# zhangrengang/SubPhaser

Measured on AMD Instinct MI355X. Metric: genome Gbases/s k-mer+enrichment, wheat k=15 1Mb windows, higher is better.
Workload: dtype u32

## Files before the change

### subphaser_amd/csrc/sp_map.h

```cpp
#pragma once
#include "sp_device.h"

#ifndef MAP_BLOOM_MAX_BITS
#define MAP_BLOOM_MAX_BITS 25
#endif
#ifndef MAP_BLOOM_MIN_BITS
#define MAP_BLOOM_MIN_BITS 12
#endif
#ifndef MAP_FILL_MAX
#define MAP_FILL_MAX 0.40
#endif
#define MAP_BLOOM_CORE 0x100
#define MAP_BLOOM_NBITS(nb) ((nb) & 0xFF)
#define MAP_RUNS 0x200
#ifndef MAP_RUNS_R
#define MAP_RUNS_R 2
#endif
#ifndef MAP_RUNS_P
#define MAP_RUNS_P 3
#endif
struct map_bloom_probe {
    uint32_t word, bits;
};
__host__ __device__ __forceinline__ uint32_t map_core_hash(uint64_t t) {
    uint32_t x = (uint32_t)t ^ (uint32_t)(t >> 32);
    x *= 0x9E3779B1u;
    x ^= x >> 15;
    return x * 0x85EBCA6Bu;
}
__host__ __device__ __forceinline__ uint32_t map_core_word(uint32_t hmin , int nbits) {
    const uint32_t n = ~hmin;
    const uint32_t sq = (uint32_t)(((unsigned long long)n * (unsigned long long)n) >> 32);
    return (~sq) >> (32 - (MAP_BLOOM_NBITS(nbits) - 5));
}
__host__ __device__ __forceinline__ uint32_t map_bloom_bits3(uint64_t x64, uint32_t &h) {
    const uint32_t x = (uint32_t)x64 ^ (uint32_t)(x64 >> 32);
    h = x * 0x9E3779B1u;
    const uint32_t h2 = x * 0x85EBCA6Bu;
    return (1u << ((h >> 7) & 31u)) | (1u << ((h >> 2) & 31u)) | (1u << (h2 >> 27));
}
__host__ __device__ __forceinline__ map_bloom_probe map_bloom(uint64_t x64, int k, int nbits) {
    map_bloom_probe p;
    uint32_t h;
    p.bits = map_bloom_bits3(x64, h);
    if (!(nbits & MAP_BLOOM_CORE) || k < 5) {
        p.word = h >> (32 - (MAP_BLOOM_NBITS(nbits) - 5));
        return p;
    }
    const int cb = 2 * (k - 3);
    const uint64_t smask = (1ULL << cb) - 1ULL;
    const uint64_t a = x64 >> 4, b = x64 & smask;
    const uint64_t ar = sp_revcomp(a, k - 3), br = sp_revcomp(b, k - 3);
    const uint32_t ha = map_core_hash(a < ar ? a : ar), hb = map_core_hash(b < br ? b : br);
    p.word = map_core_word(ha < hb ? ha : hb, nbits);
    return p;
}
__device__ __forceinline__ bool map_bloom_test(const uint32_t *__restrict__ bloom, int nbits, int k, uint64_t x) {
    const map_bloom_probe p = map_bloom(x, k, nbits);
    return (bloom[p.word] & p.bits) == p.bits;
}

template <typename KeyT, typename KP, typename F>
__device__ __forceinline__ void map_pair_scan(const uint32_t *__restrict__ pk, const uint32_t *__restrict__ nm,
                                              int64_t s0, const KP &kp, const uint32_t *__restrict__ bloom,
                                              int nbits, F &&hit) {
    bool pairhit = false;
    const KeyT m1mask = (KeyT)(kp.kmask >> 2);
    sp_scan_unit_all<SP_UNIT, KeyT>(pk, nm, s0, kp, [&](int64_t start, KeyT fwd, KeyT rc, bool valid_k, bool valid_k1) {
        if (!(start & 1)) {
            pairhit = false;
            if (valid_k1) {
                const KeyT mf = fwd & m1mask, mr = rc >> 2;
                pairhit = map_bloom_test(bloom, nbits, kp.k, (uint64_t)(mf < mr ? mf : mr));
            }
        }
        if (pairhit && valid_k) hit(start, fwd, rc);
    });
}

#define MAP_PAIR_MAX_SG 7

struct map_pair_loc {
    uint32_t idx;
    int field;
};
__host__ __device__ __forceinline__ map_pair_loc map_pair_loc_prefix(uint64_t o, int k) {
    map_pair_loc r;
    const uint32_t b = (uint32_t)(o & 3ULL);
    if (k == 1) { r.idx = 0; r.field = 4 + (int)b; return r; }
    const uint64_t p = o >> 2, pc = sp_revcomp(p, k - 1);
    if (p <= pc) { r.idx = (uint32_t)p; r.field = 4 + (int)b; }
    else { r.idx = (uint32_t)pc; r.field = 3 - (int)b; }
    return r;
}
__host__ __device__ __forceinline__ map_pair_loc map_pair_loc_suffix(uint64_t o, int k) {
    map_pair_loc r;
    const uint32_t b = (uint32_t)(o >> (2 * (k - 1))) & 3u;
    if (k == 1) { r.idx = 0; r.field = (int)b; return r; }
    const uint64_t m1mask = (1ULL << (2 * (k - 1))) - 1ULL;
    const uint64_t x = o & m1mask, xc = sp_revcomp(x, k - 1);
    if (x <= xc) { r.idx = (uint32_t)x; r.field = (int)b; }
    else { r.idx = (uint32_t)xc; r.field = 7 - (int)b; }
    return r;
}

#define MAP_CT_FIELD 3
#define MAP_CT_ANY 0x6DB6DBu
#define MAP_CT_PAYLOAD 0xFFFFFFu
#define MAP_CT_OVF (1u << 24)
#define MAP_CT_MAX_TAG_BITS 2
struct map_ptab {
    uint32_t *direct;
    uint4 *buckets;
    unsigned long long *ovf;
    uint32_t ovf_mask;
    int sb, tb;
};
__host__ __device__ __forceinline__ uint32_t map_ct_mix(uint32_t x, int kb) {
    const uint32_t m = kb >= 32 ? 0xFFFFFFFFu : ((1u << kb) - 1u);
    uint32_t h = (x * 0x9E3779B1u) & m;
    h ^= h >> ((kb + 1) / 2);
    h = (h * 0x85EBCA6Bu) & m;
    h ^= h >> ((kb + 1) / 2);
    return h;
}
__host__ __device__ __forceinline__ uint32_t map_ct_ovf_home(uint32_t x) { return (x * 0xC2B2AE35u) >> 7; }
struct map_ct_key {
    uint32_t bucket, tag, kid;
};
__host__ __device__ __forceinline__ map_ct_key map_ct_key_of(const map_ptab &T, uint32_t t, uint32_t side, uint32_t e) {
    const uint32_t h = map_ct_mix(t, T.sb);
    map_ct_key r;
    r.bucket = h >> T.tb;
    r.tag = ((h & ((1u << T.tb) - 1u)) << 5) | (side << 4) | e;
    r.kid = (t << 5) | (side << 4) | e;
    return r;
}
struct map_ct_hit {
    uint32_t fields, loc;
};
__device__ __forceinline__ map_ct_hit map_ct_find(const map_ptab &T, const uint4 &B, const map_ct_key &q) {
    map_ct_hit r;
// ... 129 lines not shown
```

### subphaser_amd/csrc/sp_map.hip

```cpp
#include "sp_device.h"
#include "sp_internal.h"
#include "sp_map.h"

__global__ void __launch_bounds__(256)
k4_pair_filter(const unsigned long long *__restrict__ keys, int64_t n, int k, uint32_t *__restrict__ bloom, int nbits) {
    int64_t i = (int64_t)blockIdx.x * blockDim.x + threadIdx.x;
    if (i >= n) return;
    const uint64_t key = keys[i];
    uint64_t pre = 0, suf = 0;
    if (k > 1) {
        const uint64_t m1mask = (k - 1 >= 32) ? ~0ULL : ((1ULL << (2 * (k - 1))) - 1ULL);
        pre = key >> 2;
        suf = key & m1mask;
        const uint64_t rpre = sp_revcomp(pre, k - 1), rsuf = sp_revcomp(suf, k - 1);
        pre = pre < rpre ? pre : rpre;
        suf = suf < rsuf ? suf : rsuf;
    }
    const map_bloom_probe p = map_bloom(pre, k, nbits);
    atomicOr(&bloom[p.word], p.bits);
    const map_bloom_probe q = map_bloom(suf, k, nbits);
    atomicOr(&bloom[q.word], q.bits);
}

__global__ void __launch_bounds__(256)
k4_filter_fill(const uint32_t *__restrict__ bloom, int64_t n_words, unsigned long long *__restrict__ out) {
    __shared__ unsigned long long red[16];
    unsigned long long c = 0;
    for (int64_t i = (int64_t)blockIdx.x * blockDim.x + threadIdx.x; i < n_words; i += (int64_t)gridDim.x * blockDim.x)
        c += __popc(bloom[i]);
    unsigned long long t = sp_block_sum_u64(c, red);
    if (threadIdx.x == 0 && t) atomicAdd(out, t);
}

__global__ void __launch_bounds__(256)
k4_labels(const unsigned long long *__restrict__ keys, const uint8_t *__restrict__ sg, int64_t n,
          sp_kparams kp, uint8_t *__restrict__ label) {
    int64_t i = (int64_t)blockIdx.x * blockDim.x + threadIdx.x;
    if (i >= n) return;
    label[sp_slot_of_key(keys[i], kp)] = (uint8_t)(1u + sg[i]);
}

__global__ void __launch_bounds__(256)
k4_pair_table(const unsigned long long *__restrict__ keys, const uint8_t *__restrict__ sg, int64_t n, int k,
              uint32_t *__restrict__ ptab) {
    int64_t i = (int64_t)blockIdx.x * blockDim.x + threadIdx.x;
    if (i >= n) return;
    const uint64_t key = keys[i];
    const uint32_t l = 1u + sg[i];
    const map_pair_loc a = map_pair_loc_prefix(key, k), b = map_pair_loc_suffix(key, k);
    atomicOr(&ptab[a.idx], l << (4 * a.field));
    atomicOr(&ptab[b.idx], l << (4 * b.field));
    const uint64_t r = sp_revcomp(key, k);
    const map_pair_loc c = map_pair_loc_prefix(r, k), d = map_pair_loc_suffix(r, k);
    atomicOr(&ptab[c.idx], l << (4 * c.field));
    atomicOr(&ptab[d.idx], l << (4 * d.field));
}

__global__ void __launch_bounds__(256)
k4_pair_clear(const unsigned long long *__restrict__ keys, int64_t n, int k, uint32_t *__restrict__ ptab) {
    int64_t i = (int64_t)blockIdx.x * blockDim.x + threadIdx.x;
    if (i >= n) return;
    const uint64_t key = keys[i], r = sp_revcomp(key, k);
    ptab[map_pair_loc_prefix(key, k).idx] = 0u;
    ptab[map_pair_loc_suffix(key, k).idx] = 0u;
    ptab[map_pair_loc_prefix(r, k).idx] = 0u;
    ptab[map_pair_loc_suffix(r, k).idx] = 0u;
}

__global__ void __launch_bounds__(256)
k4_pair_seen(const unsigned long long *__restrict__ keys, int64_t n, int k, const uint32_t *__restrict__ ptab,
             unsigned long long *__restrict__ out) {
    __shared__ unsigned long long red[16];
    unsigned long long c = 0;
    for (int64_t i = (int64_t)blockIdx.x * blockDim.x + threadIdx.x; i < n; i += (int64_t)gridDim.x * blockDim.x) {
        const uint64_t key = keys[i], r = sp_revcomp(key, k);
        const map_pair_loc a = map_pair_loc_prefix(key, k), b = map_pair_loc_suffix(key, k);
        const map_pair_loc e = map_pair_loc_prefix(r, k), f = map_pair_loc_suffix(r, k);
        const uint32_t seen = ((ptab[a.idx] >> (4 * a.field)) | (ptab[b.idx] >> (4 * b.field)) |
                               (ptab[e.idx] >> (4 * e.field)) | (ptab[f.idx] >> (4 * f.field))) & 8u;
        c += seen ? 1 : 0;
    }
    unsigned long long t = sp_block_sum_u64(c, red);
    if (threadIdx.x == 0 && t) atomicAdd(out, t);
}

__device__ __forceinline__ void map_ct_insert(const map_ptab &T, const map_ct_key &q, uint32_t bits, unsigned long long *fail) {
    uint32_t *e = reinterpret_cast<uint32_t *>(T.buckets + q.bucket);
    const uint32_t fresh = (q.tag << 25) | bits;
    for (int j = 0; j < 4; j++) {
        const int i = (int)((q.tag + (uint32_t)j) & 3u);
        const uint32_t old = atomicCAS(&e[i], 0u, fresh);
        if (old == 0u) return;
        if ((old >> 25) == q.tag && (old & MAP_CT_PAYLOAD)) {
            atomicOr(&e[i], bits);
            return;
        }
    }
    atomicOr(&e[0], MAP_CT_OVF);
    const unsigned long long mine = ((unsigned long long)(q.kid + 1u) << 32) | bits;
    uint32_t i = map_ct_ovf_home(q.kid) & T.ovf_mask;
    for (uint32_t probes = 0; probes <= T.ovf_mask; probes++) {
        const unsigned long long old = atomicCAS(&T.ovf[i], 0ULL, mine);
        if (old == 0ULL) {
            atomicAdd(fail + 1, 1ULL);
// ... 26 lines not shown
    __shared__ unsigned long long red[16];
    unsigned long long c = 0;
    for (int64_t i = (int64_t)blockIdx.x * blockDim.x + threadIdx.x; i < n; i += (int64_t)gridDim.x * blockDim.x) {
        const uint64_t o2[2] = {keys[i], sp_revcomp(keys[i], k)};
        uint32_t seen = 0;
        for (int r = 0; r < 2; r++) {
            map_ct_site st[4];
            const int ns = map_ct_sites(o2[r], k, st);
            for (int j = 0; j < ns; j++) {
                const map_ct_key q = map_ct_key_of(T, st[j].t, st[j].side, st[j].e);
                const uint4 B = T.buckets[q.bucket];
                seen |= (map_ct_find(T, B, q).fields >> (MAP_CT_FIELD * st[j].field)) & 4u;
            }
        }
        c += seen ? 1 : 0;
    }
    unsigned long long t = sp_block_sum_u64(c, red);
    if (threadIdx.x == 0 && t) atomicAdd(out, t);
}

struct map_chrom_desc {
    const uint32_t *pk, *pm, *nm;
    int64_t n_units;
    int64_t nslots;
    int64_t range0;
    int *counts;
    unsigned long long *n_mapped;
};

#ifndef MAP_MIN_WAVES
#define MAP_MIN_WAVES 8
#endif
#ifndef MAP2_QI
#define MAP2_QI 1
#endif
struct map_quad_win {
    uint32_t V1, V2, xf1, xr1, xf2, xr2;
};
__device__ __forceinline__ map_quad_win map_quad_windows(uint32_t l0, uint32_t l1, uint32_t m0, uint32_t m1, int r ,
                                                         int sh, uint32_t m1mask) {
    map_quad_win q;
    const uint32_t W1 = __builtin_amdgcn_alignbit(l1, l0, 2 * r), W2 = __builtin_amdgcn_alignbit(l1, l0, 2 * r + 4);
    const unsigned long long mm = ((unsigned long long)m0 << 32) | m1;
    q.V1 = (uint32_t)((mm << (2 * r)) >> 32);
    q.V2 = (uint32_t)((mm << (2 * r + 4)) >> 32);
    q.xf1 = (q.V1 >> sh) & m1mask;
    q.xr1 = (~W1 >> 2) & m1mask;
    q.xf2 = (q.V2 >> sh) & m1mask;
    q.xr2 = (~W2 >> 2) & m1mask;
    return q;
}
template <int TABLE>
__device__ __forceinline__ void map_unit_scan64(const uint32_t *__restrict__ pk, const uint32_t *__restrict__ pm,
                                                const uint32_t *__restrict__ nm, int64_t s0, const sp_kparams32 &kp,
                                                const uint32_t *__restrict__ bloom, int nbits, const map_ptab &T,
                                                unsigned long long lab[3], const map_unit_lds &U,
                                                unsigned long long cm = ~0ULL ) {
    constexpr int FW = TABLE ? MAP_CT_FIELD : 4;
    constexpr uint32_t LBL = TABLE ? 3u : 7u, SEEN = TABLE ? 4u : 8u, FMASK = TABLE ? 7u : 15u;
    constexpr uint32_t ANY = TABLE ? MAP_CT_ANY : 0x77777777u;
    constexpr int NP = TABLE ? 2 : 3, ROUND_W = TABLE ? MAP2_ROUND_W : 2;
    unsigned long long ok_k, ok_x;
    {
        const uint64_t badA = sp_bad_starts64(nm, s0, kp.k - 1), badB = sp_bad_starts64(nm, s0 + 32, kp.k - 1);
        const uint64_t invA = (uint64_t)nm[s0 >> 5] | ((uint64_t)nm[(s0 >> 5) + 1] << 32);
        const uint64_t invB = (uint64_t)nm[(s0 >> 5) + 1] | ((uint64_t)nm[(s0 >> 5) + 2] << 32);
        const uint32_t kA = ~(uint32_t)(badA | (invA >> (kp.k - 1))), kB = ~(uint32_t)(badB | (invB >> (kp.k - 1)));
        const uint32_t xA = ~(uint32_t)(badA >> 1), xB = ~(uint32_t)(badB >> 1);
        ok_k = (unsigned long long)kA | ((unsigned long long)kB << 32);
        ok_x = (unsigned long long)xA | ((unsigned long long)xB << 32);
    }
    if (__all((ok_x & 0x5555555555555555ULL) == 0)) return;
    const unsigned long long here = __ballot(1);
    const int n_here = __popcll(here);
    const int me = (int)__builtin_amdgcn_mbcnt_hi((uint32_t)(here >> 32), __builtin_amdgcn_mbcnt_lo((uint32_t)here, 0u));
    const int tid = (int)threadIdx.x, lane = tid & 63, wave0 = tid & ~63;
    uint32_t *sw = U.words + tid;
    uint16_t *queue = U.queue + (tid >> 6) * MAP_QCAP(TABLE);
    const int64_t w0 = s0 >> 4;
    const uint4 la = *reinterpret_cast<const uint4 *>(pk + w0);
    uint32_t l0 = la.x, l1 = la.y, l2 = la.z, l3 = la.w, l4 = pk[w0 + 4];
#if SP_DERIVE_PM
    (void)pm;
    uint32_t m0 = sp_msb_of_lsb(l0), m1 = sp_msb_of_lsb(l1), m2 = sp_msb_of_lsb(l2), m3 = sp_msb_of_lsb(l3), m4 = sp_msb_of_lsb(l4);
#else
    const uint4 ma = *reinterpret_cast<const uint4 *>(pm + w0);
    uint32_t m0 = ma.x, m1 = ma.y, m2 = ma.z, m3 = ma.w, m4 = pm[w0 + 4];
#endif
    {
        const unsigned long long okc = ok_k & cm;
        sw[0 * MAP_BLOCK] = l0; sw[1 * MAP_BLOCK] = l1; sw[2 * MAP_BLOCK] = l2; sw[3 * MAP_BLOCK] = l3; sw[4 * MAP_BLOCK] = l4;
        sw[5 * MAP_BLOCK] = (uint32_t)okc; sw[6 * MAP_BLOCK] = (uint32_t)(okc >> 32);
#pragma unroll
        for (int bit = 0; bit < NP; bit++) U.planes[bit * MAP_BLOCK + tid] = 0ULL;
    }
    const int sh = 32 - 2 * kp.k, sh1 = 30 - 2 * kp.k;
    const uint32_t m1mask = kp.kmask >> 2;
    const int sb = T.sb;
    const uint32_t smask = TABLE ? ((1u << sb) - 1u) : 0u;
    const bool core = (nbits & MAP_BLOOM_CORE) && kp.k >= 5;
    const uint32_t cmask = kp.k >= 5 ? ((1u << (2 * (kp.k - 3))) - 1u) : 0u;
    const int wsh = 32 - (MAP_BLOOM_NBITS(nbits) - 5);
    uint32_t last_wi = 0xFFFFFFFFu, last_w = 0u;
    uint32_t h_carry = 0u;
    static_assert(MAP2_QI == 1, "the runs rule decides a quad from the filter's answer for the quad before it");
    const bool runs = (nbits & MAP_RUNS) != 0;
    uint32_t run = 0u;
#pragma unroll 1
    for (int wr = 0; wr < 4; wr += ROUND_W) {
        uint32_t qn = 0;
#pragma unroll 1
        for (int w = wr; w < wr + ROUND_W; w++) {
#pragma unroll 1
            for (int r0 = 0; r0 < 16; r0 += 4 * MAP2_QI) {
                uint32_t bt1[MAP2_QI], bt2[MAP2_QI], wi1[MAP2_QI], wi2[MAP2_QI], f1[MAP2_QI], f2[MAP2_QI];
                bool v1[MAP2_QI], v2[MAP2_QI], need1[MAP2_QI], need2[MAP2_QI], guess[MAP2_QI];
                uint32_t lw = last_wi;
#pragma unroll
                for (int q = 0; q < MAP2_QI; q++) {
                    const int r = r0 + 4 * q, j = 16 * w + r;
                    const map_quad_win Q = map_quad_windows(l0, l1, m0, m1, r, sh, m1mask);
                    const uint32_t c1 = Q.xf1 < Q.xr1 ? Q.xf1 : Q.xr1, c2 = Q.xf2 < Q.xr2 ? Q.xf2 : Q.xr2;
                    uint32_t h1, h2;
                    bt1[q] = map_bloom_bits3((uint64_t)c1, h1);
                    bt2[q] = map_bloom_bits3((uint64_t)c2, h2);
                    const uint32_t okx = (uint32_t)(ok_x >> j);
                    v1[q] = okx & 1u;
                    v2[q] = okx & 4u;
                    if (core) {
                        const uint32_t tb_f = Q.xf1 & cmask, tb_r = Q.xr1 >> 4, tc_f = Q.xf2 & cmask, tc_r = Q.xr2 >> 4;
                        uint32_t ha = h_carry;
                        if (j == 0) {
                            const uint32_t ta_f = Q.xf1 >> 4, ta_r = Q.xr1 & cmask;
                            ha = map_core_hash((uint64_t)(ta_f < ta_r ? ta_f : ta_r));
                        }
                        const uint32_t hb = map_core_hash((uint64_t)(tb_f < tb_r ? tb_f : tb_r));
                        const uint32_t hc = map_core_hash((uint64_t)(tc_f < tc_r ? tc_f : tc_r));
                        h_carry = hc;
                        wi1[q] = map_core_word(ha < hb ? ha : hb, nbits);
                        wi2[q] = map_core_word(hb < hc ? hb : hc, nbits);
                    } else {
                        wi1[q] = h1 >> wsh;
                        wi2[q] = h2 >> wsh;
                    }
                    guess[q] = runs && v1[q] && v2[q] && run - (uint32_t)MAP_RUNS_R < (uint32_t)MAP_RUNS_P;
                    need1[q] = !guess[q] && v1[q] && wi1[q] != lw;
                    need2[q] = !guess[q] && v2[q] && wi2[q] != (v1[q] ? wi1[q] : lw);
                    f1[q] = f2[q] = 0;
                    if (need1[q]) f1[q] = bloom[wi1[q]];
                    if (need2[q]) f2[q] = bloom[wi2[q]];
                    if (!guess[q]) {
                        if (v2[q]) lw = wi2[q];
                        else if (v1[q]) lw = wi1[q];
                    }
                }
                last_wi = lw;
#pragma unroll
                for (int q = 0; q < MAP2_QI; q++) {
                    const int j = 16 * w + r0 + 4 * q;
                    const uint32_t wd1 = v1[q] ? (need1[q] ? f1[q] : last_w) : 0u;
                    const uint32_t wd2 = v2[q] ? (need2[q] ? f2[q] : (v1[q] ? wd1 : last_w)) : 0u;
                    if (!guess[q]) {
                        if (v2[q]) last_w = wd2;
                        else if (v1[q]) last_w = wd1;
                    }
                    const bool cand1 = guess[q] || (wd1 & bt1[q]) == bt1[q], cand2 = guess[q] || (wd2 & bt2[q]) == bt2[q];
                    run = guess[q] ? run + 1u : (cand1 && cand2) ? (run < (uint32_t)MAP_RUNS_R ? run + 1u : (uint32_t)MAP_RUNS_R) : 0u;
                    const unsigned long long bal = __ballot(cand1 || cand2);
                    if (cand1 || cand2)
                        queue[qn + __builtin_amdgcn_mbcnt_hi((uint32_t)(bal >> 32), __builtin_amdgcn_mbcnt_lo((uint32_t)bal, 0u))] =
                            (uint16_t)((uint32_t)lane | ((uint32_t)(j >> 2) << 6) | (cand1 ? 0x400u : 0u) | (cand2 ? 0x800u : 0u));
                    qn += (uint32_t)__popcll(bal);
                }
            }
            l0 = l1; l1 = l2; l2 = l3; l3 = l4;
            m0 = m1; m1 = m2; m2 = m3; m3 = m4;
        }
        __builtin_amdgcn_fence(__ATOMIC_RELEASE, "wavefront");
        __builtin_amdgcn_wave_barrier();
        __builtin_amdgcn_fence(__ATOMIC_ACQUIRE, "wavefront");
        for (uint32_t e0 = (uint32_t)me; e0 < qn; e0 += (uint32_t)(MAP2_P2 * n_here)) {
            bool live[MAP2_P2], cand1[MAP2_P2], cand2[MAP2_P2], sfw[MAP2_P2];
            int owner[MAP2_P2], jj[MAP2_P2];
            map_quad_win Q[MAP2_P2];
            uint32_t okk[MAP2_P2], e1[MAP2_P2], e2[MAP2_P2];
            map_ct_key k1[MAP2_P2], k2[MAP2_P2];
            uint4 B[MAP2_P2];
#pragma unroll
            for (int p = 0; p < MAP2_P2; p++) {
                const uint32_t e = e0 + (uint32_t)(p * n_here);
                live[p] = e < qn;
                const uint32_t ent = live[p] ? (uint32_t)queue[e] : 0u;
                const int qi = (int)((ent >> 6) & 15u), w = qi >> 2;
                owner[p] = wave0 + (int)(ent & 63u);
                jj[p] = 4 * qi;
                cand1[p] = ent & 0x400u;
                cand2[p] = ent & 0x800u;
                const uint32_t *ow = U.words + owner[p];
                const uint32_t ola = ow[w * MAP_BLOCK], olb = ow[(w + 1) * MAP_BLOCK];
                Q[p] = map_quad_windows(ola, olb, sp_msb_of_lsb(ola), sp_msb_of_lsb(olb), jj[p] & 15, sh, m1mask);
                okk[p] = ow[(5 + (w >> 1)) * MAP_BLOCK] >> (jj[p] & 31);
                e1[p] = e2[p] = 0;
                sfw[p] = false;
                B[p] = make_uint4(0u, 0u, 0u, 0u);
                if (TABLE) {
                    const uint32_t s_f = cand1[p] ? (Q[p].xf1 & smask) : (Q[p].xf2 >> 4), s_r = cand1[p] ? (Q[p].xr1 >> 4) : (Q[p].xr2 & smask);
                    sfw[p] = s_f <= s_r;
                    const uint32_t t = sfw[p] ? s_f : s_r;
                    k1[p] = map_ct_key_of(T, t, sfw[p] ? 0u : 1u, sfw[p] ? (Q[p].xf1 >> sb) : (Q[p].xr1 & 15u));
                    k2[p] = map_ct_key_of(T, t, sfw[p] ? 1u : 0u, sfw[p] ? (Q[p].xf2 & 15u) : (Q[p].xr2 >> sb));
                    if (live[p]) B[p] = T.buckets[k1[p].bucket];
                } else {
                    if (cand1[p]) e1[p] = T.direct[Q[p].xf1 < Q[p].xr1 ? Q[p].xf1 : Q[p].xr1];
                    if (cand2[p]) e2[p] = T.direct[Q[p].xf2 < Q[p].xr2 ? Q[p].xf2 : Q[p].xr2];
                }
            }
#pragma unroll
            for (int p = 0; p < MAP2_P2; p++) {
                if (!live[p]) continue;
                const int j = jj[p];
                uint32_t loc1 = Q[p].xf1 < Q[p].xr1 ? Q[p].xf1 : Q[p].xr1, loc2 = Q[p].xf2 < Q[p].xr2 ? Q[p].xf2 : Q[p].xr2;
                bool fw1 = Q[p].xf1 <= Q[p].xr1, fw2 = Q[p].xf2 <= Q[p].xr2;
                if (TABLE) {
                    if (cand1[p]) {
                        const map_ct_hit h = map_ct_find(T, B[p], k1[p]);
                        e1[p] = h.fields;
                        loc1 = h.loc;
                    }
                    if (cand2[p]) {
                        const map_ct_hit h = map_ct_find(T, B[p], k2[p]);
                        e2[p] = h.fields;
                        loc2 = h.loc;
                    }
                    fw1 = fw2 = sfw[p];
                }
#pragma unroll
                for (int h = 0; h < 2; h++) {
                    const uint32_t ee = h ? e2[p] : e1[p];
                    if (!(ee & ANY)) continue;
                    const uint32_t V = h ? Q[p].V2 : Q[p].V1;
                    const bool fw = h ? fw2 : fw1;
                    const uint32_t b0 = V >> 30, b1 = (V >> sh1) & 3u;
                    const int f0 = fw ? (int)b0 : 7 - (int)b0, f1 = fw ? 4 + (int)b1 : 3 - (int)b1;
                    const uint32_t cnt2 = okk[p] >> (2 * h);
                    const uint32_t v0 = (cnt2 & 1u) ? (ee >> (FW * f0)) & FMASK : 0u;
                    const uint32_t v1 = (cnt2 & 2u) ? (ee >> (FW * f1)) & FMASK : 0u;
                    const uint32_t two = (v0 & LBL) | ((v1 & LBL) << 8);
                    if (!two) continue;
#pragma unroll
                    for (int bit = 0; bit < NP; bit++) {
                        const unsigned long long b2 = (unsigned long long)(((two >> bit) & 1u) | (((two >> (8 + bit)) & 1u) << 1));
                        if (b2) atomicOr(&U.planes[bit * MAP_BLOCK + owner[p]], b2 << (j + 2 * h));
                    }
                    uint32_t mark = 0;
                    if ((v0 & LBL) && !(v0 & SEEN)) mark |= SEEN << (FW * f0);
                    if ((v1 & LBL) && !(v1 & SEEN)) mark |= SEEN << (FW * f1);
                    if (mark) {
                        if (TABLE) map_ct_mark(T, h ? loc2 : loc1, mark);
                        else atomicOr(&T.direct[h ? loc2 : loc1], mark);
// ... 977 lines not shown
```

### subphaser_amd/csrc/sp_sparse.hip

```cpp
#include <algorithm>
#include <cstring>
#include <utility>
#include <rocprim/rocprim.hpp>

#include "sp_device.h"
#include "sp_internal.h"
#include "sp_lists.h"
#include "sp_map.h"

__global__ void __launch_bounds__(256)
sps_keygen(const uint32_t *__restrict__ pk, const uint32_t *__restrict__ nm, int64_t n_units, sp_kparams kp,
           unsigned long long *__restrict__ keys ,
           unsigned long long *__restrict__ n_valid) {
    __shared__ unsigned long long red[16];
    unsigned long long nv = 0;
    for (int64_t u = (int64_t)blockIdx.x * blockDim.x + threadIdx.x; u < n_units;
         u += (int64_t)gridDim.x * blockDim.x) {
        sp_scan_unit64<SP_UNIT>(pk, nm, u * SP_UNIT, kp, [&](int64_t start, uint64_t fwd, uint64_t rc) {
            keys[start] = fwd < rc ? fwd : rc;
            nv++;
        });
    }
    unsigned long long t = sp_block_sum_u64(nv, red);
    if (threadIdx.x == 0 && t) atomicAdd(n_valid, t);
// ... 328 lines not shown
    unsigned long long c = 0;
    for (int64_t i = (int64_t)blockIdx.x * blockDim.x + threadIdx.x; i < n; i += (int64_t)gridDim.x * blockDim.x) {
        const uint64_t o2[2] = {keys[i], sp_revcomp(keys[i], k)};
        uint32_t seen = 0;
        for (int r = 0; r < 2; r++) {
            sq_site st[4];
            const int ns = sq_sites(o2[r], k, st);
            for (int j = 0; j < ns; j++) {
                const sq_key q = sq_key_of(T, st[j].t, st[j].side, st[j].e);
                const ulonglong2 *bp = reinterpret_cast<const ulonglong2 *>(T.buckets + 4 * q.bucket);
                seen |= (sq_find(T, bp[0], bp[1], q.bucket, q.tag, st[j].t, (st[j].side << 4) | st[j].e).fields >> (SQ_FIELD * st[j].field)) & 4u;
            }
        }
        c += seen ? 1 : 0;
    }
    const unsigned long long t = sp_block_sum_u64(c, red);
    if (threadIdx.x == 0 && t) atomicAdd(out, t);
}

struct map_pair_win {
    uint64_t xf, xr;
    uint32_t b0, b1;
};
__device__ __forceinline__ map_pair_win map_pair_window(uint32_t la, uint32_t lb, uint32_t lc, uint32_t ma, uint32_t mb, uint32_t mc,
                                                        int rr, int k, int sh, uint64_t m1mask) {
    map_pair_win q;
    const uint64_t W = (uint64_t)__builtin_amdgcn_alignbit(lb, la, 2 * rr) | ((uint64_t)__builtin_amdgcn_alignbit(lc, lb, 2 * rr) << 32);
    const unsigned long long mA = ((unsigned long long)ma << 32) | mb, mB = ((unsigned long long)mb << 32) | mc;
    const uint64_t V = (((mA << (2 * rr)) >> 32) << 32) | ((mB << (2 * rr)) >> 32);
    q.b0 = (uint32_t)(V >> 62);
    q.xf = (V >> sh) & m1mask;
    q.xr = (~W >> 2) & m1mask;
    const int pb = rr + k;
    q.b1 = (((pb >> 4) == 1 ? lb : lc) >> (2 * (pb & 15))) & 3u;
    return q;
}
template <int TABLE>
__device__ __forceinline__ void map_unit_scan64_h(const uint32_t *__restrict__ pk, const uint32_t *__restrict__ pm,
                                                  const uint32_t *__restrict__ nm, int64_t s0, const sp_kparams &kp,
                                                  const uint32_t *__restrict__ bloom, int nbits,
                                                  unsigned long long *__restrict__ htab, uint64_t hmask, const sq_tab &T,
                                                  unsigned long long lab[3], const map_unit_lds &U,
                                                  unsigned long long cm = ~0ULL ) {
    constexpr int FW = TABLE ? SQ_FIELD : 4;
    constexpr uint32_t LBL = TABLE ? 3u : 7u, SEEN = TABLE ? 4u : 8u, FMASK = TABLE ? 7u : 15u;
    constexpr uint32_t ANY = TABLE ? (uint32_t)SQ_ANY : 0x77777777u;
    constexpr int NP = TABLE ? 2 : 3, ROUND_W = TABLE ? MAP2_ROUND_W : 2;
    unsigned long long ok_k, ok_x;
    {
        const uint64_t badA = sp_bad_starts64(nm, s0, kp.k - 1), badB = sp_bad_starts64(nm, s0 + 32, kp.k - 1);
        const uint64_t invA = (uint64_t)nm[s0 >> 5] | ((uint64_t)nm[(s0 >> 5) + 1] << 32);
        const uint64_t invB = (uint64_t)nm[(s0 >> 5) + 1] | ((uint64_t)nm[(s0 >> 5) + 2] << 32);
        const uint32_t kA = ~(uint32_t)(badA | (invA >> (kp.k - 1))), kB = ~(uint32_t)(badB | (invB >> (kp.k - 1)));
        const uint32_t xA = ~(uint32_t)(badA >> 1), xB = ~(uint32_t)(badB >> 1);
        ok_k = ((unsigned long long)kA | ((unsigned long long)kB << 32)) & cm;
        ok_x = (unsigned long long)xA | ((unsigned long long)xB << 32);
    }
    if (__all((ok_x & 0x5555555555555555ULL) == 0)) return;
    const unsigned long long here = __ballot(1);
    const int n_here = __popcll(here);
    const int me = (int)__builtin_amdgcn_mbcnt_hi((uint32_t)(here >> 32), __builtin_amdgcn_mbcnt_lo((uint32_t)here, 0u));
    const int tid = (int)threadIdx.x, lane = tid & 63, wave0 = tid & ~63;
    uint32_t *sw = U.words + tid;
    uint16_t *queue = U.queue + (tid >> 6) * MAP_QCAP(TABLE);
    const int64_t w0 = s0 >> 4;
    const uint4 la = *reinterpret_cast<const uint4 *>(pk + w0);
    uint32_t l0 = la.x, l1 = la.y, l2 = la.z, l3 = la.w, l4 = pk[w0 + 4], l5 = pk[w0 + 5];
#if SP_DERIVE_PM
    (void)pm;
    uint32_t m0 = sp_msb_of_lsb(l0), m1 = sp_msb_of_lsb(l1), m2 = sp_msb_of_lsb(l2), m3 = sp_msb_of_lsb(l3), m4 = sp_msb_of_lsb(l4),
             m5 = sp_msb_of_lsb(l5);
#else
    const uint4 ma = *reinterpret_cast<const uint4 *>(pm + w0);
    uint32_t m0 = ma.x, m1 = ma.y, m2 = ma.z, m3 = ma.w, m4 = pm[w0 + 4], m5 = pm[w0 + 5];
#endif
    sw[0 * MAP_BLOCK] = l0; sw[1 * MAP_BLOCK] = l1; sw[2 * MAP_BLOCK] = l2; sw[3 * MAP_BLOCK] = l3; sw[4 * MAP_BLOCK] = l4; sw[5 * MAP_BLOCK] = l5;
    sw[6 * MAP_BLOCK] = (uint32_t)ok_k; sw[7 * MAP_BLOCK] = (uint32_t)(ok_k >> 32);
#pragma unroll
    for (int bit = 0; bit < NP; bit++) U.planes[bit * MAP_BLOCK + tid] = 0ULL;
    const int sh = 64 - 2 * kp.k;
    const uint64_t m1mask = kp.kmask >> 2;
    const bool core = (nbits & MAP_BLOOM_CORE) != 0;
    const uint64_t cmask = (1ULL << (2 * (kp.k - 3))) - 1ULL;
    const int wsh = 32 - (MAP_BLOOM_NBITS(nbits) - 5);
    uint32_t last_wi = 0xFFFFFFFFu, last_w = 0u;
    uint32_t h_carry = 0u;
#pragma unroll 1
    for (int wr = 0; wr < 4; wr += ROUND_W) {
        uint32_t qn = 0;
#pragma unroll 1
        for (int w = wr; w < wr + ROUND_W; w++) {
#pragma unroll 1
            for (int r = 0; r < 16; r += 4) {
                const int j = 16 * w + r;
                const map_pair_win A = map_pair_window(l0, l1, l2, m0, m1, m2, r, kp.k, sh, m1mask);
                const map_pair_win B = map_pair_window(l0, l1, l2, m0, m1, m2, r + 2, kp.k, sh, m1mask);
                uint32_t hx1, hx2;
                const uint32_t bt1 = map_bloom_bits3(A.xf < A.xr ? A.xf : A.xr, hx1), bt2 = map_bloom_bits3(B.xf < B.xr ? B.xf : B.xr, hx2);
                uint32_t wi1, wi2;
                if (core) {
                    const uint64_t tb_f = A.xf & cmask, tb_r = A.xr >> 4, tc_f = B.xf & cmask, tc_r = B.xr >> 4;
                    uint32_t ha = h_carry;
                    if (j == 0) {
                        const uint64_t ta_f = A.xf >> 4, ta_r = A.xr & cmask;
                        ha = map_core_hash(ta_f < ta_r ? ta_f : ta_r);
                    }
                    const uint32_t hb = map_core_hash(tb_f < tb_r ? tb_f : tb_r), hc = map_core_hash(tc_f < tc_r ? tc_f : tc_r);
                    h_carry = hc;
                    wi1 = map_core_word(ha < hb ? ha : hb, nbits);
                    wi2 = map_core_word(hb < hc ? hb : hc, nbits);
                } else {
                    wi1 = hx1 >> wsh;
                    wi2 = hx2 >> wsh;
                }
                const bool v1 = (ok_x >> j) & 1ULL, v2 = (ok_x >> (j + 2)) & 1ULL;
                const bool need1 = v1 && wi1 != last_wi;
                const bool need2 = v2 && wi2 != (v1 ? wi1 : last_wi);
                uint32_t f1 = 0, f2 = 0;
                if (need1) f1 = bloom[wi1];
                if (need2) f2 = bloom[wi2];
                const uint32_t wd1 = v1 ? (need1 ? f1 : last_w) : 0u;
                const uint32_t wd2 = v2 ? (need2 ? f2 : (v1 ? wd1 : last_w)) : 0u;
                if (v2) { last_wi = wi2; last_w = wd2; }
                else if (v1) { last_wi = wi1; last_w = wd1; }
                const bool cand1 = (wd1 & bt1) == bt1, cand2 = (wd2 & bt2) == bt2;
                const unsigned long long bal = __ballot(cand1 || cand2);
                if (cand1 || cand2)
                    queue[qn + __builtin_amdgcn_mbcnt_hi((uint32_t)(bal >> 32), __builtin_amdgcn_mbcnt_lo((uint32_t)bal, 0u))] =
                        (uint16_t)((uint32_t)lane | ((uint32_t)(j >> 2) << 6) | (cand1 ? 0x400u : 0u) | (cand2 ? 0x800u : 0u));
                qn += (uint32_t)__popcll(bal);
            }
            l0 = l1; l1 = l2; l2 = l3; l3 = l4; l4 = l5;
            m0 = m1; m1 = m2; m2 = m3; m3 = m4; m4 = m5;
        }
        __builtin_amdgcn_fence(__ATOMIC_RELEASE, "wavefront");
        __builtin_amdgcn_wave_barrier();
        __builtin_amdgcn_fence(__ATOMIC_ACQUIRE, "wavefront");
        for (uint32_t e0 = (uint32_t)me; e0 < qn; e0 += (uint32_t)n_here) {
            const uint32_t ent = queue[e0];
            const int owner = wave0 + (int)(ent & 63u), qi = (int)((ent >> 6) & 15u), j = 4 * qi, w = qi >> 2, r = j & 15;
            const bool cand[2] = {(ent & 0x400u) != 0u, (ent & 0x800u) != 0u};
            const uint32_t *ow = U.words + owner;
            const uint32_t oa = ow[w * MAP_BLOCK], ob = ow[(w + 1) * MAP_BLOCK], oc = ow[(w + 2) * MAP_BLOCK];
            const uint32_t okq = ow[(6 + (w >> 1)) * MAP_BLOCK] >> (j & 31);
            const uint32_t pa = sp_msb_of_lsb(oa), pb_ = sp_msb_of_lsb(ob), pc = sp_msb_of_lsb(oc);
            const map_pair_win Pw[2] = {map_pair_window(oa, ob, oc, pa, pb_, pc, r, kp.k, sh, m1mask),
                                        map_pair_window(oa, ob, oc, pa, pb_, pc, r + 2, kp.k, sh, m1mask)};
            uint32_t e[2] = {0u, 0u};
            uint32_t loc[2] = {0u, 0u};
            uint64_t slot[2] = {0, 0};
            bool fwd_[2] = {Pw[0].xf <= Pw[0].xr, Pw[1].xf <= Pw[1].xr};
            if (TABLE) {
                const uint64_t s_f = cand[0] ? (Pw[0].xf & cmask) : (Pw[1].xf >> 4), s_r = cand[0] ? (Pw[0].xr >> 4) : (Pw[1].xr & cmask);
                const bool sfw = s_f <= s_r;
                const uint64_t t = sfw ? s_f : s_r;
                const uint64_t hm = sq_mix(t, T.sb);
                const uint64_t bucket = hm >> T.tb, tagb = (hm & ((1ULL << T.tb) - 1ULL)) << 5;
                const uint32_t se1 = (sfw ? 0u : 16u) | (uint32_t)(sfw ? (Pw[0].xf >> T.sb) : (Pw[0].xr & 15ULL));
                const uint32_t se2 = (sfw ? 16u : 0u) | (uint32_t)(sfw ? (Pw[1].xf & 15ULL) : (Pw[1].xr >> T.sb));
                const ulonglong2 *bp = reinterpret_cast<const ulonglong2 *>(T.buckets + 4 * bucket);
                const ulonglong2 B0 = bp[0], B1 = bp[1];
                if (cand[0]) {
                    const sq_hit hh = sq_find(T, B0, B1, bucket, tagb | se1, t, se1);
                    e[0] = hh.fields;
                    loc[0] = hh.loc;
                }
                if (cand[1]) {
                    const sq_hit hh = sq_find(T, B0, B1, bucket, tagb | se2, t, se2);
                    e[1] = hh.fields;
                    loc[1] = hh.loc;
                }
                fwd_[0] = fwd_[1] = sfw;
            } else {
#pragma unroll
                for (int h = 0; h < 2; h++)
                    if (cand[h]) e[h] = sps_pair_get(Pw[h].xf < Pw[h].xr ? Pw[h].xf : Pw[h].xr, htab, hmask, slot[h]);
            }
#pragma unroll
            for (int h = 0; h < 2; h++) {
                if (!(e[h] & ANY)) continue;
                const bool fw = fwd_[h];
                const int f0 = fw ? (int)Pw[h].b0 : 7 - (int)Pw[h].b0, f1 = fw ? 4 + (int)Pw[h].b1 : 3 - (int)Pw[h].b1;
                const uint32_t okk = okq >> (2 * h);
                const uint32_t v0 = (okk & 1u) ? (e[h] >> (FW * f0)) & FMASK : 0u;
                const uint32_t v1 = (okk & 2u) ? (e[h] >> (FW * f1)) & FMASK : 0u;
                const uint32_t two = (v0 & LBL) | ((v1 & LBL) << 8);
                if (!two) continue;
#pragma unroll
                for (int bit = 0; bit < NP; bit++) {
                    const unsigned long long b2 = (unsigned long long)(((two >> bit) & 1u) | (((two >> (8 + bit)) & 1u) << 1));
                    if (b2) atomicOr(&U.planes[bit * MAP_BLOCK + owner], b2 << (j + 2 * h));
                }
                uint32_t mark = 0;
                if ((v0 & LBL) && !(v0 & SEEN)) mark |= SEEN << (FW * f0);
                if ((v1 & LBL) && !(v1 & SEEN)) mark |= SEEN << (FW * f1);
                if (mark) {
                    if (TABLE) sq_mark(T, loc[h], mark);
                    else atomicOr(&htab[2 * slot[h] + 1], (unsigned long long)mark);
                }
            }
        }
        __builtin_amdgcn_fence(__ATOMIC_RELEASE, "wavefront");
        __builtin_amdgcn_wave_barrier();
        __builtin_amdgcn_fence(__ATOMIC_ACQUIRE, "wavefront");
    }
#pragma unroll
    for (int bit = 0; bit < NP; bit++) lab[bit] = U.planes[bit * MAP_BLOCK + tid];
}
// ... 649 lines not shown
```

Baseline: 156.8.

## Generalise blocked Bloom filter to configurable 32/64/128-bit blocks

Moves the Bloom filter helpers into a shared header and lets the block size (32, 64 or 128 bits) and number of hash bits per key be chosen at compile time. Wider blocks are loaded with vector loads and filled with 64-bit atomics, and the fill limit scales with the hash count. The intent is a lower false-positive rate at the same memory, so fewer candidates reach the exact lookup stage. The default stays a 32-bit block, and the derived-msb path now computes the msb plane on the fly per step instead of precomputing five registers, which cuts register pressure.

```diff
diff --git a/subphaser_amd/csrc/sp_bloom.h b/subphaser_amd/csrc/sp_bloom.h
--- /dev/null
+++ b/subphaser_amd/csrc/sp_bloom.h
@@ -0,0 +1,114 @@
+#pragma once
+#include <stdint.h>
+#if defined(__HIPCC__)
+#define SP_BLOOM_HD __host__ __device__ __forceinline__
+#else
+#define SP_BLOOM_HD static inline
+#endif
+
+#ifndef MAP_BLOOM_MAX_BITS
+#define MAP_BLOOM_MAX_BITS 25
+#endif
+#ifndef MAP_BLOOM_MIN_BITS
+#define MAP_BLOOM_MIN_BITS 12
+#endif
+#ifndef MAP_BLOOM_BLOCK
+#define MAP_BLOOM_BLOCK 32
+#endif
+#ifndef MAP_BLOOM_K
+#define MAP_BLOOM_K (MAP_BLOOM_BLOCK == 32 ? 3 : MAP_BLOOM_BLOCK == 64 ? 4 : 5)
+#endif
+#define MAP_BLOOM_LOG (MAP_BLOOM_BLOCK == 32 ? 5 : MAP_BLOOM_BLOCK == 64 ? 6 : 7)
+#define MAP_BLOOM_WORDS (MAP_BLOOM_BLOCK / 32)
+static_assert(MAP_BLOOM_BLOCK == 32 || MAP_BLOOM_BLOCK == 64 || MAP_BLOOM_BLOCK == 128, "MAP_BLOOM_BLOCK: 32, 64 or 128");
+static_assert(MAP_BLOOM_BLOCK == 32 ? MAP_BLOOM_K == 3 : (MAP_BLOOM_K == 4 || MAP_BLOOM_K == 5), "MAP_BLOOM_K: 3 at 32 bits, 4 or 5 above");
+static_assert(MAP_BLOOM_MIN_BITS > MAP_BLOOM_LOG && MAP_BLOOM_MAX_BITS - MAP_BLOOM_LOG < 32, "block index: 1 .. 31 bits");
+#ifndef MAP_FILL_MAX
+#define MAP_FILL_MAX (MAP_BLOOM_K == 3 ? 0.40 : MAP_BLOOM_K == 4 ? 0.494 : 0.573)
+#endif
+#define MAP_BLOOM_CORE 0x100
+#define MAP_BLOOM_NBITS(nb) ((nb) & 0xFF)
+
+struct map_bloom_blk {
+    uint32_t w[MAP_BLOOM_WORDS];
+};
+struct map_bloom_probe {
+    uint32_t block;
+    map_bloom_blk bits;
+};
+SP_BLOOM_HD bool map_bloom_pass(const map_bloom_blk &have, const map_bloom_blk &want) {
+    bool ok = true;
+    for (int i = 0; i < MAP_BLOOM_WORDS; i++) ok = ok && (have.w[i] & want.w[i]) == want.w[i];
+    return ok;
+}
+SP_BLOOM_HD uint64_t map_bloom_revcomp(uint64_t x, int k) {
+    x = ~x;
+    x = ((x >> 2) & 0x3333333333333333ULL) | ((x & 0x3333333333333333ULL) << 2);
+    x = ((x >> 4) & 0x0F0F0F0F0F0F0F0FULL) | ((x & 0x0F0F0F0F0F0F0F0FULL) << 4);
+    x = ((x >> 8) & 0x00FF00FF00FF00FFULL) | ((x & 0x00FF00FF00FF00FFULL) << 8);
+    x = ((x >> 16) & 0x0000FFFF0000FFFFULL) | ((x & 0x0000FFFF0000FFFFULL) << 16);
+    x = (x >> 32) | (x << 32);
+    return x >> (64 - 2 * k);
+}
+SP_BLOOM_HD uint32_t map_core_hash(uint64_t t) {
+    uint32_t x = (uint32_t)t ^ (uint32_t)(t >> 32);
+    x *= 0x9E3779B1u;
+    x ^= x >> 15;
+    return x * 0x85EBCA6Bu;
+}
+SP_BLOOM_HD uint32_t map_core_word(uint32_t hmin , int nbits) {
+    const uint32_t n = ~hmin;
+    const uint32_t sq = (uint32_t)(((unsigned long long)n * (unsigned long long)n) >> 32);
+    return (~sq) >> (32 - (MAP_BLOOM_NBITS(nbits) - MAP_BLOOM_LOG));
+}
+SP_BLOOM_HD uint32_t map_hash_word(uint32_t h, int nbits) { return h >> (32 - (MAP_BLOOM_NBITS(nbits) - MAP_BLOOM_LOG)); }
+SP_BLOOM_HD uint32_t map_bloom_sel(uint64_t x64, uint32_t &h) {
+    const uint32_t x = (uint32_t)x64 ^ (uint32_t)(x64 >> 32);
+    h = x * 0x9E3779B1u;
+    const uint32_t h2 = x * 0x85EBCA6Bu;
+#if MAP_BLOOM_BLOCK == 32
+    return (1u << ((h >> 7) & 31u)) | (1u << ((h >> 2) & 31u)) | (1u << (h2 >> 27));
+#else
+    return h2;
+#endif
+}
+SP_BLOOM_HD map_bloom_blk map_bloom_mask(uint32_t sel) {
+    map_bloom_blk b;
+#if MAP_BLOOM_BLOCK == 32
+    b.w[0] = sel;
+#elif MAP_BLOOM_BLOCK == 64
+    b.w[0] = (1u << (sel >> 28)) | (0x10000u << ((sel >> 24) & 15u));
+#if MAP_BLOOM_K == 4
+    b.w[1] = (1u << ((sel >> 20) & 15u)) | (0x10000u << ((sel >> 16) & 15u));
+#else
+    b.w[1] = (1u << ((sel >> 20) & 15u)) | (0x10000u << ((sel >> 17) & 7u)) | (0x1000000u << ((sel >> 14) & 7u));
+#endif
+#else
+    b.w[0] = 1u << (sel >> 27);
+    b.w[1] = 1u << ((sel >> 22) & 31u);
+    b.w[2] = 1u << ((sel >> 17) & 31u);
+#if MAP_BLOOM_K == 4
+    b.w[3] = 1u << ((sel >> 12) & 31u);
+#else
+    b.w[3] = (1u << ((sel >> 13) & 15u)) | (0x10000u << ((sel >> 9) & 15u));
+#endif
+#endif
+    return b;
+}
+SP_BLOOM_HD map_bloom_blk map_bloom_bits(uint64_t x64, uint32_t &h) { return map_bloom_mask(map_bloom_sel(x64, h)); }
+SP_BLOOM_HD map_bloom_probe map_bloom(uint64_t x64, int k, int nbits) {
+    map_bloom_probe p;
+    uint32_t h;
+    p.bits = map_bloom_bits(x64, h);
+    if (!(nbits & MAP_BLOOM_CORE) || k < 5) {
+        p.block = map_hash_word(h, nbits);
+        return p;
+    }
+    const int cb = 2 * (k - 3);
+    const uint64_t smask = (1ULL << cb) - 1ULL;
+    const uint64_t a = x64 >> 4, b = x64 & smask;
+    const uint64_t ar = map_bloom_revcomp(a, k - 3), br = map_bloom_revcomp(b, k - 3);
+    const uint32_t ha = map_core_hash(a < ar ? a : ar), hb = map_core_hash(b < br ? b : br);
+    p.block = map_core_word(ha < hb ? ha : hb, nbits);
+    return p;
+}
diff --git a/subphaser_amd/csrc/sp_map.h b/subphaser_amd/csrc/sp_map.h
--- a/subphaser_amd/csrc/sp_map.h
+++ b/subphaser_amd/csrc/sp_map.h
@@ -1,17 +1,7 @@
 #pragma once
 #include "sp_device.h"
-
-#ifndef MAP_BLOOM_MAX_BITS
-#define MAP_BLOOM_MAX_BITS 25
-#endif
-#ifndef MAP_BLOOM_MIN_BITS
-#define MAP_BLOOM_MIN_BITS 12
-#endif
-#ifndef MAP_FILL_MAX
-#define MAP_FILL_MAX 0.40
-#endif
-#define MAP_BLOOM_CORE 0x100
-#define MAP_BLOOM_NBITS(nb) ((nb) & 0xFF)
+#include "sp_bloom.h"
+
 #define MAP_RUNS 0x200
 #ifndef MAP_RUNS_R
 #define MAP_RUNS_R 2
@@ -19,45 +9,22 @@
 #ifndef MAP_RUNS_P
 #define MAP_RUNS_P 3
 #endif
-struct map_bloom_probe {
-    uint32_t word, bits;
-};
-__host__ __device__ __forceinline__ uint32_t map_core_hash(uint64_t t) {
-    uint32_t x = (uint32_t)t ^ (uint32_t)(t >> 32);
-    x *= 0x9E3779B1u;
-    x ^= x >> 15;
-    return x * 0x85EBCA6Bu;
-}
-__host__ __device__ __forceinline__ uint32_t map_core_word(uint32_t hmin , int nbits) {
-    const uint32_t n = ~hmin;
-    const uint32_t sq = (uint32_t)(((unsigned long long)n * (unsigned long long)n) >> 32);
-    return (~sq) >> (32 - (MAP_BLOOM_NBITS(nbits) - 5));
-}
-__host__ __device__ __forceinline__ uint32_t map_bloom_bits3(uint64_t x64, uint32_t &h) {
-    const uint32_t x = (uint32_t)x64 ^ (uint32_t)(x64 >> 32);
-    h = x * 0x9E3779B1u;
-    const uint32_t h2 = x * 0x85EBCA6Bu;
-    return (1u << ((h >> 7) & 31u)) | (1u << ((h >> 2) & 31u)) | (1u << (h2 >> 27));
-}
-__host__ __device__ __forceinline__ map_bloom_probe map_bloom(uint64_t x64, int k, int nbits) {
-    map_bloom_probe p;
-    uint32_t h;
-    p.bits = map_bloom_bits3(x64, h);
-    if (!(nbits & MAP_BLOOM_CORE) || k < 5) {
-        p.word = h >> (32 - (MAP_BLOOM_NBITS(nbits) - 5));
-        return p;
-    }
-    const int cb = 2 * (k - 3);
-    const uint64_t smask = (1ULL << cb) - 1ULL;
-    const uint64_t a = x64 >> 4, b = x64 & smask;
-    const uint64_t ar = sp_revcomp(a, k - 3), br = sp_revcomp(b, k - 3);
-    const uint32_t ha = map_core_hash(a < ar ? a : ar), hb = map_core_hash(b < br ? b : br);
-    p.word = map_core_word(ha < hb ? ha : hb, nbits);
-    return p;
+__device__ __forceinline__ map_bloom_blk map_bloom_load(const uint32_t *__restrict__ bloom, uint32_t block) {
+    map_bloom_blk b;
+#if MAP_BLOOM_WORDS == 1
+    b.w[0] = bloom[block];
+#elif MAP_BLOOM_WORDS == 2
+    const uint2 v = reinterpret_cast<const uint2 *>(bloom)[block];
+    b.w[0] = v.x; b.w[1] = v.y;
+#else
+    const uint4 v = reinterpret_cast<const uint4 *>(bloom)[block];
+    b.w[0] = v.x; b.w[1] = v.y; b.w[2] = v.z; b.w[3] = v.w;
+#endif
+    return b;
 }
 __device__ __forceinline__ bool map_bloom_test(const uint32_t *__restrict__ bloom, int nbits, int k, uint64_t x) {
     const map_bloom_probe p = map_bloom(x, k, nbits);
-    return (bloom[p.word] & p.bits) == p.bits;
+    return map_bloom_pass(map_bloom_load(bloom, p.block), p.bits);
 }
 
 template <typename KeyT, typename KP, typename F>
diff --git a/subphaser_amd/csrc/sp_map.hip b/subphaser_amd/csrc/sp_map.hip
--- a/subphaser_amd/csrc/sp_map.hip
+++ b/subphaser_amd/csrc/sp_map.hip
@@ -17,9 +17,18 @@
         suf = suf < rsuf ? suf : rsuf;
     }
     const map_bloom_probe p = map_bloom(pre, k, nbits);
-    atomicOr(&bloom[p.word], p.bits);
     const map_bloom_probe q = map_bloom(suf, k, nbits);
-    atomicOr(&bloom[q.word], q.bits);
+#if MAP_BLOOM_WORDS == 1
+    atomicOr(&bloom[p.block], p.bits.w[0]);
+    atomicOr(&bloom[q.block], q.bits.w[0]);
+#else
+    unsigned long long *b64 = reinterpret_cast<unsigned long long *>(bloom);
+#pragma unroll
+    for (int i = 0; i < MAP_BLOOM_WORDS / 2; i++) {
+        atomicOr(&b64[(size_t)p.block * (MAP_BLOOM_WORDS / 2) + i], (unsigned long long)p.bits.w[2 * i] | ((unsigned long long)p.bits.w[2 * i + 1] << 32));
+        atomicOr(&b64[(size_t)q.block * (MAP_BLOOM_WORDS / 2) + i], (unsigned long long)q.bits.w[2 * i] | ((unsigned long long)q.bits.w[2 * i + 1] << 32));
+    }
+#endif
 }
 
 __global__ void __launch_bounds__(256)
@@ -212,7 +221,7 @@
     uint32_t l0 = la.x, l1 = la.y, l2 = la.z, l3 = la.w, l4 = pk[w0 + 4];
 #if SP_DERIVE_PM
     (void)pm;
-    uint32_t m0 = sp_msb_of_lsb(l0), m1 = sp_msb_of_lsb(l1), m2 = sp_msb_of_lsb(l2), m3 = sp_msb_of_lsb(l3), m4 = sp_msb_of_lsb(l4);
+    uint32_t m0 = sp_msb_of_lsb(l0), m1 = sp_msb_of_lsb(l1);
 #else
     const uint4 ma = *reinterpret_cast<const uint4 *>(pm + w0);
     uint32_t m0 = ma.x, m1 = ma.y, m2 = ma.z, m3 = ma.w, m4 = pm[w0 + 4];
@@ -230,8 +239,8 @@
     const uint32_t smask = TABLE ? ((1u << sb) - 1u) : 0u;
     const bool core = (nbits & MAP_BLOOM_CORE) && kp.k >= 5;
     const uint32_t cmask = kp.k >= 5 ? ((1u << (2 * (kp.k - 3))) - 1u) : 0u;
-    const int wsh = 32 - (MAP_BLOOM_NBITS(nbits) - 5);
-    uint32_t last_wi = 0xFFFFFFFFu, last_w = 0u;
+    uint32_t last_wi = 0xFFFFFFFFu;
+    map_bloom_blk last_w = {};
     uint32_t h_carry = 0u;
     static_assert(MAP2_QI == 1, "the runs rule decides a quad from the filter's answer for the quad before it");
     const bool runs = (nbits & MAP_RUNS) != 0;
@@ -243,7 +252,9 @@
         for (int w = wr; w < wr + ROUND_W; w++) {
 #pragma unroll 1
             for (int r0 = 0; r0 < 16; r0 += 4 * MAP2_QI) {
-                uint32_t bt1[MAP2_QI], bt2[MAP2_QI], wi1[MAP2_QI], wi2[MAP2_QI], f1[MAP2_QI], f2[MAP2_QI];
+                uint32_t wi1[MAP2_QI], wi2[MAP2_QI];
+                uint32_t bt1[MAP2_QI], bt2[MAP2_QI];
+                map_bloom_blk f1[MAP2_QI], f2[MAP2_QI];
                 bool v1[MAP2_QI], v2[MAP2_QI], need1[MAP2_QI], need2[MAP2_QI], guess[MAP2_QI];
                 uint32_t lw = last_wi;
 #pragma unroll
@@ -252,8 +263,8 @@
                     const map_quad_win Q = map_quad_windows(l0, l1, m0, m1, r, sh, m1mask);
                     const uint32_t c1 = Q.xf1 < Q.xr1 ? Q.xf1 : Q.xr1, c2 = Q.xf2 < Q.xr2 ? Q.xf2 : Q.xr2;
                     uint32_t h1, h2;
-                    bt1[q] = map_bloom_bits3((uint64_t)c1, h1);
-                    bt2[q] = map_bloom_bits3((uint64_t)c2, h2);
+                    bt1[q] = map_bloom_sel((uint64_t)c1, h1);
+                    bt2[q] = map_bloom_sel((uint64_t)c2, h2);
                     const uint32_t okx = (uint32_t)(ok_x >> j);
                     v1[q] = okx & 1u;
                     v2[q] = okx & 4u;
@@ -270,15 +281,16 @@
                         wi1[q] = map_core_word(ha < hb ? ha : hb, nbits);
                         wi2[q] = map_core_word(hb < hc ? hb : hc, nbits);
                     } else {
-                        wi1[q] = h1 >> wsh;
-                        wi2[q] = h2 >> wsh;
+                        wi1[q] = map_hash_word(h1, nbits);
+                        wi2[q] = map_hash_word(h2, nbits);
                     }
                     guess[q] = runs && v1[q] && v2[q] && run - (uint32_t)MAP_RUNS_R < (uint32_t)MAP_RUNS_P;
                     need1[q] = !guess[q] && v1[q] && wi1[q] != lw;
                     need2[q] = !guess[q] && v2[q] && wi2[q] != (v1[q] ? wi1[q] : lw);
-                    f1[q] = f2[q] = 0;
-                    if (need1[q]) f1[q] = bloom[wi1[q]];
-                    if (need2[q]) f2[q] = bloom[wi2[q]];
+                    f1[q] = last_w;
+                    f2[q] = map_bloom_blk{};
+                    if (need1[q]) f1[q] = map_bloom_load(bloom, wi1[q]);
+                    if (need2[q]) f2[q] = map_bloom_load(bloom, wi2[q]);
                     if (!guess[q]) {
                         if (v2[q]) lw = wi2[q];
                         else if (v1[q]) lw = wi1[q];
@@ -288,13 +300,9 @@
 #pragma unroll
                 for (int q = 0; q < MAP2_QI; q++) {
                     const int j = 16 * w + r0 + 4 * q;
-                    const uint32_t wd1 = v1[q] ? (need1[q] ? f1[q] : last_w) : 0u;
-                    const uint32_t wd2 = v2[q] ? (need2[q] ? f2[q] : (v1[q] ? wd1 : last_w)) : 0u;
-                    if (!guess[q]) {
-                        if (v2[q]) last_w = wd2;
-                        else if (v1[q]) last_w = wd1;
-                    }
-                    const bool cand1 = guess[q] || (wd1 & bt1[q]) == bt1[q], cand2 = guess[q] || (wd2 & bt2[q]) == bt2[q];
+                    const map_bloom_blk wd1 = f1[q], wd2 = need2[q] ? f2[q] : wd1;
+                    last_w = wd2;
+                    const bool cand1 = guess[q] || (v1[q] && map_bloom_pass(wd1, map_bloom_mask(bt1[q]))), cand2 = guess[q] || (v2[q] && map_bloom_pass(wd2, map_bloom_mask(bt2[q])));
                     run = guess[q] ? run + 1u : (cand1 && cand2) ? (run < (uint32_t)MAP_RUNS_R ? run + 1u : (uint32_t)MAP_RUNS_R) : 0u;
                     const unsigned long long bal = __ballot(cand1 || cand2);
                     if (cand1 || cand2)
@@ -304,7 +312,11 @@
                 }
             }
             l0 = l1; l1 = l2; l2 = l3; l3 = l4;
+#if SP_DERIVE_PM
+            m0 = m1; m1 = sp_msb_of_lsb(l1);
+#else
             m0 = m1; m1 = m2; m2 = m3; m3 = m4;
+#endif
         }
         __builtin_amdgcn_fence(__ATOMIC_RELEASE, "wavefront");
         __builtin_amdgcn_wave_barrier();
diff --git a/subphaser_amd/csrc/sp_sparse.hip b/subphaser_amd/csrc/sp_sparse.hip
--- a/subphaser_amd/csrc/sp_sparse.hip
+++ b/subphaser_amd/csrc/sp_sparse.hip
@@ -434,8 +434,8 @@
     const uint64_t m1mask = kp.kmask >> 2;
     const bool core = (nbits & MAP_BLOOM_CORE) != 0;
     const uint64_t cmask = (1ULL << (2 * (kp.k - 3))) - 1ULL;
-    const int wsh = 32 - (MAP_BLOOM_NBITS(nbits) - 5);
-    uint32_t last_wi = 0xFFFFFFFFu, last_w = 0u;
+    uint32_t last_wi = 0xFFFFFFFFu;
+    map_bloom_blk last_w = {};
     uint32_t h_carry = 0u;
 #pragma unroll 1
     for (int wr = 0; wr < 4; wr += ROUND_W) {
@@ -448,7 +448,7 @@
                 const map_pair_win A = map_pair_window(l0, l1, l2, m0, m1, m2, r, kp.k, sh, m1mask);
                 const map_pair_win B = map_pair_window(l0, l1, l2, m0, m1, m2, r + 2, kp.k, sh, m1mask);
                 uint32_t hx1, hx2;
-                const uint32_t bt1 = map_bloom_bits3(A.xf < A.xr ? A.xf : A.xr, hx1), bt2 = map_bloom_bits3(B.xf < B.xr ? B.xf : B.xr, hx2);
+                const uint32_t bt1 = map_bloom_sel(A.xf < A.xr ? A.xf : A.xr, hx1), bt2 = map_bloom_sel(B.xf < B.xr ? B.xf : B.xr, hx2);
                 uint32_t wi1, wi2;
                 if (core) {
                     const uint64_t tb_f = A.xf & cmask, tb_r = A.xr >> 4, tc_f = B.xf & cmask, tc_r = B.xr >> 4;
@@ -462,20 +462,20 @@
                     wi1 = map_core_word(ha < hb ? ha : hb, nbits);
                     wi2 = map_core_word(hb < hc ? hb : hc, nbits);
                 } else {
-                    wi1 = hx1 >> wsh;
-                    wi2 = hx2 >> wsh;
+                    wi1 = map_hash_word(hx1, nbits);
+                    wi2 = map_hash_word(hx2, nbits);
                 }
                 const bool v1 = (ok_x >> j) & 1ULL, v2 = (ok_x >> (j + 2)) & 1ULL;
                 const bool need1 = v1 && wi1 != last_wi;
                 const bool need2 = v2 && wi2 != (v1 ? wi1 : last_wi);
-                uint32_t f1 = 0, f2 = 0;
-                if (need1) f1 = bloom[wi1];
-                if (need2) f2 = bloom[wi2];
-                const uint32_t wd1 = v1 ? (need1 ? f1 : last_w) : 0u;
-                const uint32_t wd2 = v2 ? (need2 ? f2 : (v1 ? wd1 : last_w)) : 0u;
+                map_bloom_blk f1 = {}, f2 = {};
+                if (need1) f1 = map_bloom_load(bloom, wi1);
+                if (need2) f2 = map_bloom_load(bloom, wi2);
+                const map_bloom_blk wd1 = v1 ? (need1 ? f1 : last_w) : map_bloom_blk{};
+                const map_bloom_blk wd2 = v2 ? (need2 ? f2 : (v1 ? wd1 : last_w)) : map_bloom_blk{};
                 if (v2) { last_wi = wi2; last_w = wd2; }
                 else if (v1) { last_wi = wi1; last_w = wd1; }
-                const bool cand1 = (wd1 & bt1) == bt1, cand2 = (wd2 & bt2) == bt2;
+                const bool cand1 = map_bloom_pass(wd1, map_bloom_mask(bt1)), cand2 = map_bloom_pass(wd2, map_bloom_mask(bt2));
                 const unsigned long long bal = __ballot(cand1 || cand2);
                 if (cand1 || cand2)
                     queue[qn + __builtin_amdgcn_mbcnt_hi((uint32_t)(bal >> 32), __builtin_amdgcn_mbcnt_lo((uint32_t)bal, 0u))] =
```

New measurement: 156.8 (median of 2 runs). About the same (-0.0%).
